# kit4b/kit4b

Measured on AMD Instinct MI355X. Metric: Mreads/sec aligned (100 bp SE vs 3 Gbp .sfx), higher is better.
Workload: dtype u64

## Files before the change

kit4b_amd/csrc/k4_align.hip:

```cpp
#include <stdlib.h>
#include <type_traits>
#include "k4_align_common.h"

#define K4_BS(nch) ((nch) >= 16 ? 128 : 256)
template <int NCH>
struct K4Lane {
  const uint64_t* rd;
  uint32_t* ded;
  const uint32_t* sup;
  const uint64_t* ent;
  uint64_t* memo;
  static constexpr int NW = NCH + 1;
  K4_DEV uint64_t word(int s, int c) const { return rd[(s * NW + c) * K4_BS(NCH)]; }
  K4_DEV uint64_t chunk_at(int s, int o) const {
    int w = o >> 5, sh = 2 * (o & 31);
    uint64_t hi = word(s, w);
    if (!sh) return hi;
    return (hi << sh) | (word(s, w + 1) >> (64 - sh));
  }
};

struct K4Probe {
  int cmp;
  int mm;
  int fm;
  bool exc;
};

#define K4_MEMO_NONE 0ull
K4_DEV uint64_t k4d_memo_pack(int kind, uint64_t pos, int mm, int fm) {
  return ((uint64_t)kind << 62) | ((uint64_t)(fm & 0x3FFF) << 48) | ((uint64_t)(mm & 0xFF) << 40) | (pos & 0xFFFFFFFFFFull);
}

template <int NCH>
K4_DEV K4Probe k4d_probe(const K4DevIndex& ix, const K4Lane<NCH>& ln, int s, int o, int cl, int len, uint64_t p) {
  K4Probe r;
  int64_t left = (int64_t)p - o;
  {
    const int64_t st = left < 0 ? 0 : left;
    const uint64_t b0 = (uint64_t)st >> ix.sup_shift, b1 = (uint64_t)(left + len - 1) >> ix.sup_shift;
    const uint64_t v = (((uint64_t)ln.sup[(b0 >> 5) + 1] << 32) | ln.sup[b0 >> 5]) >> (b0 & 31);
    r.exc = (v & ((2ull << (b1 - b0)) - 1ull)) != 0;
    if (r.exc && ix.sup_shift != K4_EXC_SHIFT) r.exc = k4d_any_exc(ix, left, left + len);
  }
  r.cmp = 0;
  r.mm = 0;
  r.fm = len;
  const uint32_t* wp = ix.ref2 + (left >> 4);
  uint32_t sh = (uint32_t)(left & 15) * 2;
  uint32_t wv[2 * NCH + 1];
  if (NCH <= 5 && len + 15 <= 32 * NCH) {
    uint32_t even[2 * NCH];
    k4d_load_words<2 * NCH>(wp, even);
#pragma unroll
    for (int j = 0; j < 2 * NCH + 1; j++) wv[j] = j < 2 * NCH ? even[j] : 0u;
  } else if (NCH <= 5 || len > 32 * (NCH / 2))
    k4d_load_words<2 * NCH + 1>(wp, wv);
  else {
    uint32_t half[NCH + 1];
    k4d_load_words<NCH + 1>(wp, half);
#pragma unroll
    for (int j = 0; j < 2 * NCH + 1; j++) wv[j] = j < NCH + 1 ? half[j] : 0u;
  }
  bool decided = false;
#pragma unroll
  for (int c = 0; c < NCH; c++) {
    if (32 * c < len) {
      uint64_t hi = ((uint64_t)wv[2 * c] << 32) | wv[2 * c + 1];
      uint64_t refc = sh ? (hi << sh) | (wv[2 * c + 2] >> (32 - sh)) : hi;
      uint64_t rdc = ln.word(s, c);
      uint64_t x = rdc ^ refc;
      const uint64_t xr = x & k4d_range_mask(0, len - 32 * c);
      r.mm += (int)k4d_mm_count(xr);
      if (xr && r.fm == len) r.fm = 32 * c + (__clzll(xr) >> 1);
      uint64_t cm = k4d_range_mask(o - 32 * c, o + cl - 32 * c);
      if (!decided && (x & cm)) {
        r.cmp = (rdc & cm) < (refc & cm) ? -1 : 1;
        decided = true;
      }
    }
  }
  return r;
}

template <int EL, int NCH, typename KT, bool CAPTURE>
K4_DEV int k4d_lcm_fast(const K4AlignArgs& a, const K4Lane<NCH>& ln, int len, int allow_mm, int cl, int core_delta,
                        const K4ReadParams& rp, int* p_inst, int* p_low, int* p_nxt, k4_hit* hits,
                        uint32_t& n_lookup, uint32_t& n_probe, uint32_t& n_cand, bool defer_deep = false) {
  const K4DevIndex& ix = a.ix;
  if (*p_inst > rp.max_hits && *p_low == 0) return K4_HR_HITINSTS;
  if (*p_inst >= 1 && *p_low == 0 && (*p_nxt - *p_low) < rp.mm_delta) return K4_HR_MMDELTA;
  K4State st;
  if (*p_inst <= 0 || *p_low < 0 || *p_nxt < 0) {
    st.inst = *p_inst = 0;
    st.low = *p_low = allow_mm + rp.mm_delta + 1;
    st.nxt = *p_nxt = st.low;
  } else {
    st.inst = *p_inst; st.low = *p_low; st.nxt = *p_nxt;
  }
  st.cur_hit = st.inst < rp.max_hits ? st.inst : -1;
  const int max_iter = ix.max_iter;
  const int64_t n = (int64_t)ix.n;
  const int kk = min((int)ix.k, cl);
  const int tshift = 2 * ((int)ix.k - kk);
  typedef typename std::conditional<EL == 4, uint32_t, KT>::type RT;
  constexpr uint64_t NOPOS = sizeof(RT) == 4 ? 0xFFFFFFFFull : K4_KTAB64_MASK;
  int s = rp.strand == K4_STRAND_CRICK ? 1 : 0;
  const int s_end = rp.strand == K4_STRAND_WATSON ? 0 : 1;
  bool stop = false;
  for (; s <= s_end && !stop; s++) {
    const char strand_c = s ? '-' : '+';
    int n_ded = 0;
    int cur_delta = core_delta;
    int slides = 0;
    int o_next = 0;
    bool more = true;
    bool first_group = true;
    while (more && !stop) {
      constexpr int PFN = NCH == 5 ? K4_PF5 : K4_PF;
      int oo[PFN];
      RT lb0[PFN], ps0[PFN], lb1[PFN];
      uint32_t sig[PFN];
      int cnt = 0;
#pragma unroll
      for (int j = 0; j < PFN; j++) {
        oo[j] = 0; lb0[j] = 0; ps0[j] = 0; lb1[j] = 0; sig[j] = 0;
        if (cnt == j && slides < rp.max_slides && o_next <= len - cl && cur_delta > cl / 3) {
          if (o_next + cl + cur_delta > len) cur_delta = len - (o_next + cl);
          oo[j] = o_next;
          cnt++;
          slides++;
          o_next += cur_delta;
        }
      }
      more = cnt == PFN;
      bool memo_hit = false, memo_pending = false;
      int memo_mm = 0;
#pragma unroll
      for (int j = 0; j < PFN; j++) {
        if (j < cnt) {
          if (!CAPTURE && j == 0 && first_group && tshift == 0 && (sizeof(KT) == 4 || cl >= kk + 2)) {
            const uint64_t mv = ln.memo[s * K4_BS(NCH)];
            const int kind = (int)(mv >> 62), fm = (int)((mv >> 48) & 0x3FFF), mmv = (int)((mv >> 40) & 0xFF);
            if (kind == 1 || (kind == 2 && fm < cl)) continue;
            if (kind == 2 && mmv != 0xFF) {
              lb0[0] = 0; lb1[0] = 1; ps0[0] = (RT)(mv & 0xFFFFFFFFFFull);
              memo_hit = true; memo_mm = mmv;
              continue;
            }
          }
          const uint64_t code = ln.chunk_at(s, oo[j]) >> (64 - 2 * kk);
          uint64_t sub;
          {
            KT e_lb0, e_ps0, e_lb1;
            k4d_ktab_fetch<KT>(ix, code << tshift, (code + 1) << tshift, e_lb0, e_ps0, sig[j], e_lb1, sub,
                               sizeof(KT) == 8 && tshift == 0 && cl >= kk + 2);
            lb0[j] = (RT)e_lb0; ps0[j] = (RT)e_ps0; lb1[j] = (RT)e_lb1;
          }
          if (CAPTURE && defer_deep && tshift == 0 && (uint64_t)(lb1[j] - lb0[j]) > K4_DEFER_BUCKET) return K4_DEFER;
          if (a.deep_general && (!CAPTURE || a.deep_general == 1) && tshift == 0 && (uint64_t)(lb1[j] - lb0[j]) > K4_DEFER_BUCKET) return K4_NEED_SLOW;
          if (sizeof(KT) == 8 && tshift == 0 && cl >= kk + 2 && sub != K4_KTAB64_IRREGULAR) {
            uint32_t before, count;
            k4d_ktab_sub(sub, (uint32_t)(ln.chunk_at(s, oo[j] + kk) >> 60), before, count);
            if (before) ps0[j] = (RT)NOPOS;
            lb0[j] += (RT)before;
            lb1[j] = lb0[j] + (RT)count;
          }
          if (CAPTURE && j == 0 && first_group && tshift == 0) {
            if (lb1[0] == lb0[0]) ln.memo[s * K4_BS(NCH)] = k4d_memo_pack(1, 0, 0, 0);
            else memo_pending = lb1[0] == lb0[0] + 1;
          }
          if (sizeof(KT) == 4 && tshift == 0 && lb1[j] == lb0[j] + 1 && cl > kk) {
            const int nb = min(K4_SIG_BASES32, cl - kk);
            const uint32_t cb = (uint32_t)(ln.chunk_at(s, oo[j] + kk) >> 32);
            const uint32_t df = (cb ^ sig[j]) & (0xFFFFFFFFu << (32 - 2 * nb));
            if (df) {
              lb1[j] = lb0[j];
              if (CAPTURE && j == 0 && first_group) {
                ln.memo[s * K4_BS(NCH)] = k4d_memo_pack(2, (uint64_t)ps0[0], 0xFF, kk + (__clz(df) >> 1));
                memo_pending = false;
              }
            }
          }
        }
      }
      uint32_t touch = 0;
#pragma unroll
      for (int j = 0; j < PFN; j++)
        if (j < cnt && tshift == 0 && lb1[j] > lb0[j] && !(j == 0 && memo_hit) && (sizeof(KT) == 4 || (uint64_t)ps0[j] != NOPOS))
          touch |= ix.ref2[((int64_t)ps0[j] - oo[j]) >> 4];

#pragma unroll
      for (int j = 0; j < PFN; j++) {
        if (j >= cnt || stop) continue;
        const int o = oo[j];
        n_lookup++;
        int64_t lo = (int64_t)lb0[j];
        int64_t hi = (int64_t)lb1[j] - 1;
        const int64_t bucket_hi = hi;
        int64_t found = -1;
        uint64_t fpos = 0;
        int fmm = 0;
        while (lo <= hi) {
          const int64_t mid = (lo + hi) >> 1;
          const uint64_t p = (tshift == 0 && mid == (int64_t)lb0[j] && (sizeof(KT) == 4 || (uint64_t)ps0[j] != NOPOS))
                                 ? (uint64_t)ps0[j] : k4d_sa_at<EL>(ix, (uint64_t)mid);
          K4Probe pr;
          if (!CAPTURE && j == 0 && memo_hit) { pr.cmp = 0; pr.mm = memo_mm; pr.fm = len; pr.exc = false; }
          else {
            pr = k4d_probe<NCH>(ix, ln, s, o, cl, len, p);
            n_probe++;
            if (CAPTURE && j == 0 && memo_pending) ln.memo[s * K4_BS(NCH)] = k4d_memo_pack(2, p, pr.mm > 254 ? 254 : pr.mm, pr.fm);
          }
          if (pr.exc) return K4_NEED_SLOW;
          if (pr.cmp > 0) lo = mid + 1;
          else {
            if (pr.cmp == 0) { found = mid; fpos = p; fmm = pr.mm; }
            hi = mid - 1;
          }
        }
        if (found != lo) continue;
        int64_t idx = found;
        uint64_t p = fpos;
        int mm = fmm;
        int iter = 0;
        bool first = true;
        while (!max_iter || iter < max_iter) {
          if (!first) {
            if (idx >= bucket_hi || idx + 1 >= n) break;
            const uint64_t p2 = k4d_sa_at<EL>(ix, (uint64_t)idx + 1);
            if ((int64_t)p2 + cl > n) break;
            const K4Probe pr = k4d_probe<NCH>(ix, ln, s, o, cl, len, p2);
            n_probe++;
            if (pr.exc) return K4_NEED_SLOW;
            if (pr.cmp != 0) break;
            idx += 1; p = p2; mm = pr.mm;
          }
          first = false;
          if (p < (uint64_t)o) continue;
          const uint64_t left = p - (uint64_t)o;
          int e;
          uint64_t e_start, e_end;
          if (ix.n_entries <= K4_LDS_ENTRIES) {
            int lo_e = 0, hi_e = (int)ix.n_entries - 1;
            e = -1; e_start = 0; e_end = 0;
            while (hi_e >= lo_e) {
              const int mid_e = (hi_e + lo_e) >> 1;
              const uint64_t sv = ln.ent[mid_e];
              if (sv > left) { hi_e = mid_e - 1; continue; }
              const uint64_t ev = ln.ent[K4_LDS_ENTRIES + mid_e];
              if (ev >= left) { e = mid_e; e_start = sv; e_end = ev; break; }
              lo_e = mid_e + 1;
            }
          } else {
            e = k4d_map_entry(ix, left);
            e_start = e >= 0 ? ix.ent_start[e] : 0;
            e_end = e >= 0 ? ix.ent_end[e] : 0;
          }
          if (e < 0 || left + (uint64_t)len - 1 > e_end) continue;
          const uint32_t targ_id = (uint32_t)(1 + p - (uint32_t)o);
          bool dup = false;
          for (int q = 0; q < n_ded; q++) dup |= (ln.ded[q * K4_BS(NCH)] == targ_id);
          if (dup) continue;
          if (n_ded >= K4_DEDUP_CAP) return K4_NEED_SLOW;
          ln.ded[n_ded * K4_BS(NCH)] = targ_id;
          n_ded++;
          iter++;
          n_cand++;
          if (mm > allow_mm || mm >= st.nxt) continue;
          k4d_fold(st, mm, hits, rp.max_hits, ix.ent_id[e], (uint32_t)(left - e_start), len, strand_c);
          if (st.inst > rp.max_hits && st.low == 0) break;
        }
        if (st.inst > rp.max_hits && st.low == 0) stop = true;
      }
      if (touch == 0x5A5A5A5Au && len < 0) n_probe++;
      first_group = false;
    }
  }
  return k4d_lcm_result(*p_inst, *p_low, p_nxt, st, rp.mm_delta, rp.max_hits, p_inst, p_low);
}

K4_DEV uint64_t k4d_rev2(uint64_t x) {
  uint64_t y = __brevll(x);
  return ((y & 0x5555555555555555ull) << 1) | ((y >> 1) & 0x5555555555555555ull);
}

template <int NCH>
K4_DEV uint32_t k4d_pack_read(const uint8_t* __restrict__ src, int len, uint64_t* col, uint32_t& n_ns) {
  constexpr int NW = NCH + 1;
  uint32_t fl = 0;
  n_ns = 0;
  const uint32_t sh = (uint32_t)(reinterpret_cast<uintptr_t>(src) & 3);
  const uint32_t* __restrict__ src32 = reinterpret_cast<const uint32_t*>(src - sh);
  const int span = len + (int)sh;
#pragma unroll
  for (int c = 0; c < NCH; c++) {
    uint64_t acc = 0;
    if (32 * c < len) {
      uint32_t dq[9] = {0, 0, 0, 0, 0, 0, 0, 0, 0};
      if (c * 32 + 32 <= span) {
        uint32_t d8[8];
        k4d_load_words<8>(src32 + c * 8, d8);
#pragma unroll
        for (int q = 0; q < 8; q++) dq[q] = d8[q];
      } else {
#pragma unroll
        for (int q = 0; q < 8; q++)
          if (c * 32 + q * 4 < span) dq[q] = src32[c * 8 + q];
      }
      if (c * 32 + 32 < span) dq[8] = src32[c * 8 + 8];
#pragma unroll
      for (int q = 0; q < 8; q++) {
        const int base = c * 32 + q * 4;
        uint32_t d = __builtin_amdgcn_alignbyte(dq[q + 1], dq[q], sh);
        d &= 0x07070707u;
        if (base + 4 > len) d &= len > base ? (0xFFFFFFFFu >> (8 * (4 - (len - base)))) : 0u;
        const uint32_t hi4 = d & 0x04040404u;
        if (hi4) {
          const uint32_t inval = hi4 & ((d << 1) | (d << 2)) & 0x04040404u;
          if (inval) fl |= K4_RF_INVALID;
          n_ns += __popc(hi4 & ~inval);
          d &= ~(hi4 | (hi4 >> 1) | (hi4 >> 2));
        }
        acc = (acc << 8) | ((d & 3) << 6) | (((d >> 8) & 3) << 4) | (((d >> 16) & 3) << 2) | ((d >> 24) & 3);
      }
    }
    col[c * K4_BS(NCH)] = acc;
  }
  col[NCH * K4_BS(NCH)] = 0;
  if (n_ns) fl |= K4_RF_HAS_N;
#pragma unroll
  for (int c = 0; c < NCH; c++) {
    uint64_t r = 0;
    if (32 * c < len) {
      const int o = len - 32 * (c + 1);
      uint64_t f;
      if (o >= 0) {
        const int w = o >> 5, sh = 2 * (o & 31);
        const uint64_t hi = col[w * K4_BS(NCH)];
        f = sh ? (hi << sh) | (col[(w + 1) * K4_BS(NCH)] >> (64 - sh)) : hi;
      } else
        f = col[0] >> (2 * (-o));
      r = k4d_rev2(~f) & k4d_range_mask(0, len - 32 * c);
    }
    col[(NW + c) * K4_BS(NCH)] = r;
  }
  col[(NW + NCH) * K4_BS(NCH)] = 0;
  return fl;
}

template <int EL, int NCH, bool FIRST, typename KT, bool DEFER = false>
__global__ void __launch_bounds__(K4_BS(NCH), (NCH >= 16 ? K4_STEP_WAVES_LONG : NCH >= 8 ? K4_STEP_WAVES_MID : NCH == 5 ? K4_STEP_WAVES_5 : K4_STEP_WAVES)) k4k_align_step(K4AlignArgs a, int step, const uint32_t* __restrict__ in_ids,
                                                      const uint64_t* __restrict__ in_rows,
                                                      const uint32_t* __restrict__ in_count, uint32_t* __restrict__ out_ids,
                                                      uint64_t* __restrict__ out_rows, uint32_t* __restrict__ out_count) {
  extern __shared__ uint64_t lds[];
  constexpr int NW = NCH + 1;
  const int tid = threadIdx.x;
  const int lane = tid & 63;
  K4Lane<NCH> ln;
  ln.rd = lds + tid;
  ln.ded = reinterpret_cast<uint32_t*>(lds + 2 * NW * K4_BS(NCH)) + tid;
  ln.memo = lds + 2 * NW * K4_BS(NCH) + (K4_DEDUP_CAP * K4_BS(NCH)) / 2 + tid;
  uint64_t* ent_l = lds + 2 * NW * K4_BS(NCH) + (K4_DEDUP_CAP * K4_BS(NCH)) / 2 + 2 * K4_BS(NCH);
  uint32_t* sup_l = reinterpret_cast<uint32_t*>(ent_l + 2 * K4_LDS_ENTRIES);
  ln.ent = ent_l;
  ln.sup = sup_l;
  for (int q = tid; q < K4_SUP_WORDS; q += K4_BS(NCH)) sup_l[q] = a.ix.excsup[q];
  if (a.ix.n_entries <= K4_LDS_ENTRIES)
    for (int q = tid; q < (int)a.ix.n_entries; q += K4_BS(NCH)) {
      ent_l[q] = a.ix.ent_start[q];
      ent_l[K4_LDS_ENTRIES + q] = a.ix.ent_end[q];
    }
  __syncthreads();
  uint64_t* col = lds + tid;
  uint32_t n_lookup = 0, n_probe = 0, n_cand = 0, n_slow = 0, n_bases = 0, n_done = 0;
  const int64_t count = (FIRST && !(DEFER && in_ids != nullptr)) ? a.n_reads : (int64_t)*in_count;
  const int64_t stride = (int64_t)gridDim.x * K4_BS(NCH);
  uint32_t ch_cur = 0, ch_left = 0;
  const bool from_list = !FIRST || (DEFER && in_ids != nullptr);
  const bool may_defer = DEFER && FIRST && in_ids == nullptr && a.defer_ids != nullptr;
  uint32_t dch_cur = 0, dch_left = 0;
  for (int64_t jb = (int64_t)blockIdx.x * K4_BS(NCH) + (tid & ~63); jb < count; jb += stride) {
    const int64_t j = jb + lane;
    bool active = j < count;
    int64_t i = 0;
    if (active) {
      i = from_list ? (int64_t)in_ids[j] : j;
      if (from_list && (uint32_t)i == K4_NO_READ) active = false;
    }
    bool slow = false, survive = false, deferred = false;
    int ext_from = -1;
    if (active) {
      const int len = (int)a.lens[i];
      const K4ReadParams rp = k4d_read_params(a, len);
      bool skip = false;
      if (FIRST) {
        if (!from_list) {
          n_done++;
          n_bases += (uint32_t)len;
        }
        uint32_t fl = 0, n_ns = 0;
        if (len < 1 || len > 32 * NCH || len > K4_MAX_FAST_READ_LEN) {
          fl = K4_RF_TOOLONG;
          if (a.mode == 1) {
            const uint8_t* src = a.reads + a.offs[i];
            for (int q = 0; q < len; q++) {
              uint32_t b = src[q] & 7;
              if (b == 4) n_ns++; else if (b > 4) fl |= K4_RF_INVALID;
            }
          }
        } else
          fl = k4d_pack_read<NCH>(a.reads + a.offs[i], len, col, n_ns);
        if (a.mode == 1) {
          int max_ns = 0;
          if (a.kp.max_ns) max_ns = max((len * a.kp.max_ns) / 100, a.kp.max_ns);
          if ((fl & K4_RF_INVALID) || (int)n_ns > max_ns) {
            k4_read_result r = {K4_HR_SEQERRS, 0, 0, 0, K4_NAR_NS, 0};
            a.rr[i] = r;
            if (!a.sparse_hits)
              for (int q = 0; q < a.max_hits; q++) *reinterpret_cast<uint4*>(&a.hits[i * a.max_hits + q]) = make_uint4(0, 0, 0, 0);
            skip = true;
          }
        }
        slow = fl != 0 && !skip;
        if (((a.mode == 1 && a.kp.pe_mode == 4) || a.best) && !skip) slow = true;
      } else {
        const uint64_t* row = in_rows + (int64_t)j * K4_ROW_WORDS(NCH);
        {
          const k4_u64x2_a8 mv = *reinterpret_cast<const k4_u64x2_a8*>(row + 2 * NCH);
          ln.memo[0] = mv.x; ln.memo[K4_BS(NCH)] = mv.y;
        }
        uint64_t rw[2 * NCH];
#pragma unroll
        for (int c = 0; c < NCH; c++) {
          const k4_u64x2_a8 v = *reinterpret_cast<const k4_u64x2_a8*>(row + 2 * c);
          rw[2 * c] = v.x; rw[2 * c + 1] = v.y;
        }
#pragma unroll
        for (int c = 0; c < NCH; c++) {
          col[c * K4_BS(NCH)] = rw[c];
          col[(NW + c) * K4_BS(NCH)] = rw[NCH + c];
        }
        col[NCH * K4_BS(NCH)] = 0;
        col[(NW + NCH) * K4_BS(NCH)] = 0;
      }
      if (!skip && (rp.core_len < 1 || rp.max_hits < 1 || rp.max_hits > a.max_hits)) slow = true;
      if (!skip && !slow) {
        int n_esc = 0;
        if (rp.tot_mm > 0)
          for (; n_esc <= rp.tot_mm; n_esc++)
            if (len / (n_esc + rp.mm_delta) <= rp.core_len) break;
        const bool has_final = rp.tot_mm > 0 ? n_esc <= rp.tot_mm : true;
        const int n_phases = n_esc + (has_final ? 1 : 0);
        int allow, cl, delta;
        if (step < n_esc) { allow = step; cl = len / (step + rp.mm_delta); delta = cl; }
        else { allow = rp.tot_mm; cl = rp.core_len; delta = rp.core_delta; }
        k4_hit* hits = a.hits + i * a.max_hits;
        int inst = 0, low = 0, nxt = 0;
        const uint32_t c0 = n_lookup, c1 = n_probe, c2 = n_cand;
        if (FIRST) { ln.memo[0] = K4_MEMO_NONE; ln.memo[K4_BS(NCH)] = K4_MEMO_NONE; }
        int rslt = k4d_lcm_fast<EL, NCH, KT, FIRST>(a, ln, len, allow, cl, delta, rp, &inst, &low, &nxt, hits, n_lookup, n_probe, n_cand, DEFER && may_defer);
        if (rslt == K4_NEED_SLOW) {
          slow = true;
          n_lookup = c0; n_probe = c1; n_cand = c2;
        }
        else if (DEFER && rslt == K4_DEFER) {
          deferred = true;
          n_lookup = c0; n_probe = c1; n_cand = c2;
        }
        else if (rslt == 0 && step + 1 >= n_phases && a.ext_on) { slow = true; ext_from = n_phases; }
        else if (rslt != 0 || step + 1 >= n_phases) k4d_finalize(a, i, len, rp, rslt, inst, low, nxt);
        else survive = true;
      }
      if (slow) {
        k4d_push_slow(a, i, ext_from >= 0 ? ext_from : step);
        n_slow++;
      }
    }
    if (FIRST && DEFER) {
      const unsigned long long dm = __ballot(deferred);
      const uint32_t dcnt = (uint32_t)__popcll(dm);
      if (dcnt) {
        if (dcnt > dch_left) {
          for (uint32_t q = lane; q < dch_left; q += 64) a.defer_ids[dch_cur + q] = K4_NO_READ;
          uint32_t base = 0;
          if (lane == 0) base = atomicAdd(&a.ctl[K4_CTL_DEFER], (uint32_t)K4_CHUNK);
          dch_cur = __shfl(base, 0, 64);
          dch_left = K4_CHUNK;
        }
        if (deferred) a.defer_ids[dch_cur + (uint32_t)__popcll(dm & ((1ull << lane) - 1ull))] = (uint32_t)i;
        dch_cur += dcnt;
        dch_left -= dcnt;
      }
    }
    const unsigned long long m = __ballot(survive);
    const uint32_t cnt = (uint32_t)__popcll(m);
    if (cnt) {
      if (cnt > ch_left) {
        for (uint32_t q = lane; q < ch_left; q += 64) out_ids[ch_cur + q] = K4_NO_READ;
        uint32_t base = 0;
        if (lane == 0) base = atomicAdd(out_count, (uint32_t)K4_CHUNK);
        ch_cur = __shfl(base, 0, 64);
        ch_left = K4_CHUNK;
      }
      if (survive) {
        const uint32_t slot = ch_cur + (uint32_t)__popcll(m & ((1ull << lane) - 1ull));
        out_ids[slot] = (uint32_t)i;
        uint64_t* row = out_rows + (int64_t)slot * K4_ROW_WORDS(NCH);
#pragma unroll
        for (int c = 0; c < NCH; c++) {
          k4_u64x2_a8 v;
          const int w0 = 2 * c, w1 = 2 * c + 1;
          v.x = w0 < NCH ? col[w0 * K4_BS(NCH)] : col[(NW + w0 - NCH) * K4_BS(NCH)];
          v.y = w1 < NCH ? col[w1 * K4_BS(NCH)] : col[(NW + w1 - NCH) * K4_BS(NCH)];
          *reinterpret_cast<k4_u64x2_a8*>(row + 2 * c) = v;
        }
        {
          k4_u64x2_a8 mv;
          mv.x = ln.memo[0]; mv.y = ln.memo[K4_BS(NCH)];
          *reinterpret_cast<k4_u64x2_a8*>(row + 2 * NCH) = mv;
        }
      }
      ch_cur += cnt;
      ch_left -= cnt;
    }
  }
  for (uint32_t q = lane; q < ch_left; q += 64) out_ids[ch_cur + q] = K4_NO_READ;
  if (FIRST && DEFER)
    for (uint32_t q = lane; q < dch_left; q += 64) a.defer_ids[dch_cur + q] = K4_NO_READ;
  {
    unsigned long long v[6] = {n_done, n_lookup, n_probe, n_cand, n_slow, n_bases};
#pragma unroll
    for (int q = 0; q < 6; q++) {
      unsigned long long x = v[q];
      for (int d = 32; d > 0; d >>= 1) x += __shfl_down(x, d, 64);
      if (lane == 0 && x) atomicAdd(&a.counters[q], x);
    }
  }
}

static uint32_t next_pow2(uint64_t v) {
  uint32_t p = 1;
  while (p < v) p <<= 1;
  return p;
}

static size_t k4_survivor_slots(size_t cap) {
  static_assert(K4_CHUNK * 7 >= 8 * 63, "cap / 7 must cover the abandoned chunk tails");
  return cap + cap / 7 + (size_t)2048 * 4 * K4_CHUNK + K4_CHUNK;
}

static int nch_for(int max_len) {
  if (max_len <= 128) return 4;
  if (max_len <= 160) return 5;
  if (max_len <= 256) return 8;
  return 16;
}

extern "C" int k4_reserve(k4_index* ix, int64_t max_reads, int32_t max_read_len, int32_t max_hits) {
  if (!ix || max_reads < 0 || max_read_len < 1 || max_hits < 1) return K4_ERR_PARAMS;
  if (max_read_len > K4_MAX_READ_LEN) return k4_fail(ix, K4_ERR_PARAMS, "read length %d exceeds %d", max_read_len, K4_MAX_READ_LEN);
  if (max_reads >= 0xFFFFFFF0ll) return k4_fail(ix, K4_ERR_PARAMS, "at most 2^32-16 reads per batch");
  K4_HIP(ix, hipSetDevice(ix->device));
  K4Workspace& w = ix->ws;
  bool touched = false;
  int fast_len = std::min<int>(max_read_len, K4_MAX_FAST_READ_LEN);
  if (max_reads > w.cap_reads || fast_len > w.cap_len) {
    int64_t cap = std::max<int64_t>(max_reads, w.cap_reads);
    cap = (cap + 255) / 256 * 256;
    int len = std::max(fast_len, w.cap_len);
    int nch = nch_for(len);
    touched = true;
    w.cap_reads = 0;
    w.cap_len = 0;
    const size_t slots = k4_survivor_slots((size_t)cap);
    for (int b = 0; b < 2; b++) {
      K4_HIP(ix, w.ids[b].reserve(slots * 4));
      K4_HIP(ix, w.rows[b].reserve(slots * K4_ROW_WORDS(nch) * 8));
    }
    K4_HIP(ix, w.slow_list.reserve((size_t)cap * 4));
    K4_HIP(ix, w.slow_step.reserve((size_t)cap));
    K4_HIP(ix, w.huge_list.reserve((size_t)cap * 4));
    K4_HIP(ix, w.huge_step.reserve((size_t)cap));
    w.cap_reads = cap;
    w.cap_len = len;
  }
  if (!w.ctl.p) {
    touched = true;
    K4_HIP(ix, w.ctl.reserve(K4_CTL_WORDS * 4));
    K4_HIP(ix, hipMemset(w.ctl.p, 0, K4_CTL_WORDS * 4));
  }
  uint64_t nodes = ix->d.max_iter ? std::min<uint64_t>((uint64_t)ix->d.max_iter * 48, K4_MAX_IDENT_NODES) : K4_MAX_IDENT_NODES;
  uint32_t hcap = next_pow2(std::max<uint64_t>(2 * nodes + 2, 1024));
  if (!w.slow_hash.p || hcap > w.slow_hash_cap) {
    touched = true;
    const size_t words = (size_t)K4_SLOW_WAVES * K4_SMALL_HASH + (size_t)K4_HUGE_WAVES * hcap;
    const size_t bytes = words * 8 + (size_t)(K4_SLOW_WAVES + K4_HUGE_WAVES) * 4;
    K4_HIP(ix, w.slow_hash.reserve(bytes));
    K4_HIP(ix, hipMemset(w.slow_hash.p, 0, bytes));
    w.slow_hash_cap = hcap;
  }
  w.cap_hits = std::max(w.cap_hits, max_hits);
  if (touched) K4_HIP(ix, hipDeviceSynchronize());
  return K4_OK;
}

template <int EL, int NCH, typename KT>
static int launch_steps(k4_index* ix, K4AlignArgs& a, int n_steps, hipStream_t st) {
  K4Workspace& w = ix->ws;
  uint32_t* const ids[2] = {w.ids[0].as<uint32_t>(), w.ids[1].as<uint32_t>()};
  uint64_t* const rows[2] = {w.rows[0].as<uint64_t>(), w.rows[1].as<uint64_t>()};
  uint32_t* const ctl = w.ctl.as<uint32_t>();
  const size_t lds = (size_t)2 * (NCH + 1) * K4_BS(NCH) * 8 + (size_t)K4_DEDUP_CAP * K4_BS(NCH) * 4 + (size_t)2 * K4_BS(NCH) * 8 + (size_t)2 * K4_LDS_ENTRIES * 8 +
                     (size_t)K4_SUP_WORDS * 4 + 16;
  if (lds > 48 * 1024) {
    K4_HIP(ix, hipFuncSetAttribute((const void*)k4k_align_step<EL, NCH, true, KT, false>, hipFuncAttributeMaxDynamicSharedMemorySize, (int)lds));
    K4_HIP(ix, hipFuncSetAttribute((const void*)k4k_align_step<EL, NCH, true, KT, true>, hipFuncAttributeMaxDynamicSharedMemorySize, (int)lds));
    K4_HIP(ix, hipFuncSetAttribute((const void*)k4k_align_step<EL, NCH, false, KT>, hipFuncAttributeMaxDynamicSharedMemorySize, (int)lds));
  }
  const unsigned full = 256 * 8 * (256 / K4_BS(NCH));
  const bool timed = ix->timing && ix->ev_used < 4096;
  if (timed) {
    if (ix->ev_used == ix->ev0.size()) {
      hipEvent_t e0, e1, e2;
      K4_HIP(ix, hipEventCreate(&e0));
      K4_HIP(ix, hipEventCreate(&e1));
      K4_HIP(ix, hipEventCreate(&e2));
      ix->ev0.push_back(e0);
      ix->ev1.push_back(e1);
      ix->ev2.push_back(e2);
    }
    K4_HIP(ix, hipEventRecord(ix->ev0[ix->ev_used], st));
  }
  unsigned grid0 = (unsigned)std::min<int64_t>((a.n_reads + K4_BS(NCH) - 1) / K4_BS(NCH), full);
  static const int deep_mode = getenv("K4_DEEP_TO_GENERAL") ? atoi(getenv("K4_DEEP_TO_GENERAL")) : 0;
  a.deep_general = (deep_mode && ix->deep_bucket_frac >= K4_DEFER_MIN_FRAC) ? deep_mode : 0;
  if (ix->deep_bucket_frac >= K4_DEFER_MIN_FRAC && a.deep_general != 1) {
    a.defer_ids = ids[1];
    hipLaunchKernelGGL((k4k_align_step<EL, NCH, true, KT, true>), dim3(grid0), dim3(K4_BS(NCH)), lds, st, a, 0, (const uint32_t*)nullptr,
                       (const uint64_t*)nullptr, (const uint32_t*)nullptr, ids[0], rows[0], ctl + 2);
    hipLaunchKernelGGL((k4k_align_step<EL, NCH, true, KT, true>), dim3(grid0), dim3(K4_BS(NCH)), lds, st, a, 0, (const uint32_t*)ids[1],
                       (const uint64_t*)nullptr, (const uint32_t*)(ctl + K4_CTL_DEFER), ids[0], rows[0], ctl + 2);
  } else {
    a.defer_ids = nullptr;
    hipLaunchKernelGGL((k4k_align_step<EL, NCH, true, KT, false>), dim3(grid0), dim3(K4_BS(NCH)), lds, st, a, 0, (const uint32_t*)nullptr,
                       (const uint64_t*)nullptr, (const uint32_t*)nullptr, ids[0], rows[0], ctl + 2);
  }
  for (int t = 1; t < n_steps; t++) {
    const int in = (t - 1) & 1, out = t & 1;
    hipLaunchKernelGGL((k4k_align_step<EL, NCH, false, KT>), dim3(grid0), dim3(K4_BS(NCH)), lds, st, a, t, ids[in], rows[in],
                       ctl + 2 + (t - 1), ids[out], rows[out], ctl + 2 + t);
  }
  if (timed) K4_HIP(ix, hipEventRecord(ix->ev1[ix->ev_used], st));
  return K4_OK;
}

template <int EL, typename KT>
static int launch_all(k4_index* ix, K4AlignArgs& a, int max_len, int n_steps, hipStream_t st) {
  K4Workspace& w = ix->ws;
  const int nch = nch_for(std::min(max_len, K4_MAX_FAST_READ_LEN));
  if (nch > nch_for(w.cap_len)) return k4_fail(ix, K4_ERR_INTERNAL, "workspace not reserved for read length %d", max_len);
  if (n_steps < 1 || n_steps > K4_CTL_WORDS - 4) return k4_fail(ix, K4_ERR_INTERNAL, "bad phase count %d", n_steps);
  a.slow_list = w.slow_list.as<uint32_t>();
  a.slow_step = w.slow_step.as<uint8_t>();
  a.ctl = w.ctl.as<uint32_t>();
  a.counters = ix->counters.as<unsigned long long>();
  a.huge_list = w.huge_list.as<uint32_t>();
  a.huge_step = w.huge_step.as<uint8_t>();
  a.slow_hash = w.slow_hash.as<uint64_t>();
  a.slow_hash_cap = w.slow_hash_cap;
  a.slow_gen = reinterpret_cast<uint32_t*>(a.slow_hash + (size_t)K4_SLOW_WAVES * K4_SMALL_HASH + (size_t)K4_HUGE_WAVES * w.slow_hash_cap);
  a.nw = nch + 1;
  if (a.n_reads == 0) return K4_OK;
  K4_HIP(ix, hipMemsetAsync(w.ctl.p, 0, K4_CTL_WORDS * 4, st));
  int rc;
  switch (nch) {
    case 4: rc = launch_steps<EL, 4, KT>(ix, a, n_steps, st); break;
    case 5: rc = launch_steps<EL, 5, KT>(ix, a, n_steps, st); break;
    case 8: rc = launch_steps<EL, 8, KT>(ix, a, n_steps, st); break;
    default: rc = launch_steps<EL, 16, KT>(ix, a, n_steps, st); break;
  }
  if (rc != K4_OK) return rc;
  rc = k4i_launch_general(ix, a, max_len, st);
  if (rc != K4_OK) return rc;
  if (ix->timing && ix->ev_used < ix->ev0.size() && ix->ev_used < 4096) {
    K4_HIP(ix, hipEventRecord(ix->ev2[ix->ev_used], st));
    ix->ev_used++;
  }
  K4_HIP(ix, hipGetLastError());
  return K4_OK;
}

static int run_dev(k4_index* ix, K4AlignArgs& a, int max_len, void* stream) {
  K4Workspace& w = ix->ws;
  if (a.n_reads > w.cap_reads || std::min(max_len, K4_MAX_FAST_READ_LEN) > w.cap_len || a.max_hits > w.cap_hits ||
      !w.slow_hash.p || !w.ids[0].p || !w.ids[1].p || !w.rows[0].p || !w.rows[1].p || !w.slow_list.p || !w.huge_list.p || !w.ctl.p)
    return k4_fail(ix, K4_ERR_PARAMS, "k4_reserve(%lld, %d, %d) must precede the *_dev call", (long long)a.n_reads,
                   max_len, a.max_hits);
  a.ix = ix->d;
  hipStream_t st = (hipStream_t)stream;
  {
    const int mc = a.mode == 0 ? a.ap.min_chimeric_len : a.kp.min_chimeric_len;
    const int mi = a.mode == 0 ? a.ap.micro_indel_len : a.kp.micro_indel_len;
    const int ms = a.mode == 0 ? a.ap.max_splice_junct_len : a.kp.max_splice_junct_len;
    if (mc < 0 || mi < 0 || mi > 20 || ms < 0 || (ms != 0 && (ms < 25 || ms > 100000)))
      return k4_fail(ix, K4_ERR_PARAMS, "MinChimericLen / microInDelLen (0..20) / MaxSpliceJunctLen (0, 25..100000) out of range");
    a.ext_on = (mc > 0 || mi > 0 || ms > 0) ? 1 : 0;
    if ((mi > 0 || ms > 0) && !a.seg2)
      return k4_fail(ix, K4_ERR_PARAMS, "microInDel / splice phases report two segments: use the *_ext entry points (k4_seg2 output)");
    if (a.ext_on && (a.best || (a.mode == 1 && a.kp.pe_mode == 4)))
      return k4_fail(ix, K4_ERR_PARAMS, "the optional AlignReads phases cannot be combined with LocateBestMatches (-N)");
    if (a.seg2 && a.n_reads > 0) K4_HIP(ix, hipMemsetAsync(a.seg2, 0, (size_t)a.n_reads * sizeof(k4_seg2), st));
  }
  int tot_mm = a.ap.tot_mm;
  if (a.mode == 1) {
    tot_mm = a.kp.max_subs == 0 ? 0 : std::max(1, (int)(0.5 + (max_len * a.kp.max_subs) / 100.0));
    tot_mm = std::min(tot_mm, 63);
  }
  const int n_steps = tot_mm + 1;
  if (ix->d.el == 4) return ix->d.ktab64 ? launch_all<4, uint64_t>(ix, a, max_len, n_steps, st) : launch_all<4, uint32_t>(ix, a, max_len, n_steps, st);
  return ix->d.ktab64 ? launch_all<5, uint64_t>(ix, a, max_len, n_steps, st) : launch_all<5, uint32_t>(ix, a, max_len, n_steps, st);
}

static int check_align_params(k4_index* ix, const k4_align_params* p) {
  if (!p) return K4_ERR_PARAMS;
  if (p->tot_mm < 0 || p->tot_mm > 63 || p->core_len < 1 || p->core_delta < 0 || p->max_core_slides < 1 ||
      p->mm_delta < 1 || p->strand < 0 || p->strand > 2 || p->max_hits < 1 || p->max_hits > 4096)
    return k4_fail(ix, K4_ERR_PARAMS, "AlignReads parameters out of range");
  return K4_OK;
}

extern "C" int k4_align_reads_batch_dev(k4_index* ix, const k4_align_params* p, int64_t n, int32_t max_len,
                                        const void* d_reads, const void* d_offs, const void* d_lens, void* d_rslt,
                                        void* d_inst, void* d_low, void* d_nxt, void* d_hits, void* stream) {
  return k4_align_reads_ext_batch_dev(ix, p, n, max_len, d_reads, d_offs, d_lens, d_rslt, d_inst, d_low, d_nxt, d_hits, nullptr, stream);
}
extern "C" int k4_align_reads_ext_batch_dev(k4_index* ix, const k4_align_params* p, int64_t n, int32_t max_len,
                                            const void* d_reads, const void* d_offs, const void* d_lens, void* d_rslt,
                                            void* d_inst, void* d_low, void* d_nxt, void* d_hits, void* d_seg2, void* stream) {
  if (!ix) return K4_ERR_PARAMS;
  int rc = check_align_params(ix, p);
  if (rc != K4_OK) return rc;
  if (n < 0 || (n > 0 && (!d_reads || !d_offs || !d_lens || !d_rslt || !d_inst || !d_low || !d_nxt || !d_hits)))
    return k4_fail(ix, K4_ERR_PARAMS, "null buffer");
  K4AlignArgs a;
  memset(&a, 0, sizeof(a));
  a.reads = (const uint8_t*)d_reads; a.offs = (const uint64_t*)d_offs; a.lens = (const uint32_t*)d_lens;
  a.n_reads = n; a.mode = 0; a.ap = *p;
  a.rslt = (int32_t*)d_rslt; a.inst = (int32_t*)d_inst; a.low = (int32_t*)d_low; a.nxt = (int32_t*)d_nxt;
  a.hits = (k4_hit*)d_hits; a.max_hits = p->max_hits;
  a.seg2 = (k4_seg2*)d_seg2;
  return run_dev(ix, a, max_len, stream);
}

extern "C" int k4_best_matches_batch_dev(k4_index* ix, const k4_align_params* p, int64_t n, int32_t max_len, const void* d_reads,
                                         const void* d_offs, const void* d_lens, void* d_rslt, void* d_inst, void* d_hits,
                                         void* stream) {
  if (!ix) return K4_ERR_PARAMS;
  int rc = check_align_params(ix, p);
  if (rc != K4_OK) return rc;
  if (n < 0 || (n > 0 && (!d_reads || !d_offs || !d_lens || !d_rslt || !d_inst || !d_hits))) return k4_fail(ix, K4_ERR_PARAMS, "null buffer");
  K4AlignArgs a;
  memset(&a, 0, sizeof(a));
  a.reads = (const uint8_t*)d_reads; a.offs = (const uint64_t*)d_offs; a.lens = (const uint32_t*)d_lens;
  a.n_reads = n; a.mode = 0; a.best = 1; a.ap = *p;
  a.rslt = (int32_t*)d_rslt; a.inst = (int32_t*)d_inst;
  a.hits = (k4_hit*)d_hits; a.max_hits = p->max_hits;
  return run_dev(ix, a, max_len, stream);
}

static int resolve_kalign(k4_index* ix, const k4_kalign_params* p, k4_kalign_params* out) {
  if (!p) return K4_ERR_PARAMS;
  *out = *p;
  if (p->max_subs < 0 || p->max_subs > 15 || (p->min_edit_dist != 1 && p->min_edit_dist != 2) || p->max_ns < 0 ||
      p->strand < 0 || p->strand > 2 || p->max_ml < 1 || p->max_ml > 4096 || p->pe_mode < 0 || p->pe_mode > 4)
// ... 249 lines not shown
```

Measured before the change: 3191.

## Extend per-read memo with first two mismatch positions to skip reference probes

Widens the per-strand memo word so it stores the first and second mismatch positions of the first-phase seed alignment. In later phases, probes at the same reference window are settled from the memo: a known mismatch inside the core means no match, and an overlap free of mismatches means a match. This removes reference fetches and compare work in the binary search and in the bucket walk. The cost is an extra second-mismatch scan for surviving reads and a mismatch count now capped at 13, plus a sign-less compare result that is used only when lo == hi.

Measured after the change: 3029. 5.1% lower.

```diff
diff --git a/kit4b_amd/csrc/k4_align.hip b/kit4b_amd/csrc/k4_align.hip
--- a/kit4b_amd/csrc/k4_align.hip
+++ b/kit4b_amd/csrc/k4_align.hip
@@ -1,6 +1,7 @@
 #include <stdlib.h>
 #include <type_traits>
 #include "k4_align_common.h"
+#include "k4_window_memo.h"
 
 #define K4_BS(nch) ((nch) >= 16 ? 128 : 256)
 template <int NCH>
@@ -27,10 +28,6 @@
   bool exc;
 };
 
-#define K4_MEMO_NONE 0ull
-K4_DEV uint64_t k4d_memo_pack(int kind, uint64_t pos, int mm, int fm) {
-  return ((uint64_t)kind << 62) | ((uint64_t)(fm & 0x3FFF) << 48) | ((uint64_t)(mm & 0xFF) << 40) | (pos & 0xFFFFFFFFFFull);
-}
 
 template <int NCH>
 K4_DEV K4Probe k4d_probe(const K4DevIndex& ix, const K4Lane<NCH>& ln, int s, int o, int cl, int len, uint64_t p) {
@@ -81,6 +78,30 @@
     }
   }
   return r;
+}
+
+template <int NCH>
+K4_DEV int k4d_second_mismatch(const K4DevIndex& ix, const K4Lane<NCH>& ln, int s, int len, uint64_t left, int fm) {
+  const uint32_t* wp = ix.ref2 + (left >> 4);
+  const uint32_t sh = (uint32_t)(left & 15) * 2;
+#pragma nounroll
+  for (int c = fm >> 5; 32 * c < len; c++) {
+    const uint64_t hi = ((uint64_t)wp[2 * c] << 32) | wp[2 * c + 1];
+    const uint64_t refc = sh ? (hi << sh) | (wp[2 * c + 2] >> (32 - sh)) : hi;
+    const uint64_t x = (ln.word(s, c) ^ refc) & k4d_range_mask(fm + 1 - 32 * c, len - 32 * c);
+    if (x) return 32 * c + (__clzll(x) >> 1);
+  }
+  return len;
+}
+
+template <int NCH>
+K4_DEV void k4d_memo_complete(const K4DevIndex& ix, const K4Lane<NCH>& ln, int len) {
+#pragma nounroll
+  for (int s = 0; s < 2; s++) {
+    const uint64_t mv = ln.memo[s * K4_BS(NCH)];
+    if (k4wm_has_window(mv) && k4wm_mm(mv) >= 2)
+      ln.memo[s * K4_BS(NCH)] = k4wm_with_p2(mv, k4d_second_mismatch<NCH>(ix, ln, s, len, k4wm_pos(mv), k4wm_p1(mv)));
+  }
 }
 
 template <int EL, int NCH, typename KT, bool CAPTURE>
@@ -135,17 +156,16 @@
       }
       more = cnt == PFN;
       bool memo_hit = false, memo_pending = false;
-      int memo_mm = 0;
 #pragma unroll
       for (int j = 0; j < PFN; j++) {
         if (j < cnt) {
           if (!CAPTURE && j == 0 && first_group && tshift == 0 && (sizeof(KT) == 4 || cl >= kk + 2)) {
             const uint64_t mv = ln.memo[s * K4_BS(NCH)];
-            const int kind = (int)(mv >> 62), fm = (int)((mv >> 48) & 0x3FFF), mmv = (int)((mv >> 40) & 0xFF);
-            if (kind == 1 || (kind == 2 && fm < cl)) continue;
-            if (kind == 2 && mmv != 0xFF) {
-              lb0[0] = 0; lb1[0] = 1; ps0[0] = (RT)(mv & 0xFFFFFFFFFFull);
-              memo_hit = true; memo_mm = mmv;
+            const int kind = k4wm_kind(mv), mmv = k4wm_mm(mv);
+            if (kind == 1 || (kind == 2 && mmv != 0 && k4wm_p1(mv) < cl)) continue;
+            if (kind == 2 && mmv <= K4WM_MM_MAX) {
+              lb0[0] = 0; lb1[0] = 1; ps0[0] = (RT)k4wm_pos(mv);
+              memo_hit = true;
               continue;
             }
           }
@@ -167,7 +187,7 @@
             lb1[j] = lb0[j] + (RT)count;
           }
           if (CAPTURE && j == 0 && first_group && tshift == 0) {
-            if (lb1[0] == lb0[0]) ln.memo[s * K4_BS(NCH)] = k4d_memo_pack(1, 0, 0, 0);
+            if (lb1[0] == lb0[0]) ln.memo[s * K4_BS(NCH)] = k4wm_pack(1, 0, 0, 0, 0);
             else memo_pending = lb1[0] == lb0[0] + 1;
           }
           if (sizeof(KT) == 4 && tshift == 0 && lb1[j] == lb0[j] + 1 && cl > kk) {
@@ -177,7 +197,7 @@
             if (df) {
               lb1[j] = lb0[j];
               if (CAPTURE && j == 0 && first_group) {
-                ln.memo[s * K4_BS(NCH)] = k4d_memo_pack(2, (uint64_t)ps0[0], 0xFF, kk + (__clz(df) >> 1));
+                ln.memo[s * K4_BS(NCH)] = k4wm_pack_unfetched((uint64_t)ps0[0], kk + (__clz(df) >> 1));
                 memo_pending = false;
               }
             }
@@ -187,7 +207,8 @@
       uint32_t touch = 0;
 #pragma unroll
       for (int j = 0; j < PFN; j++)
-        if (j < cnt && tshift == 0 && lb1[j] > lb0[j] && !(j == 0 && memo_hit) && (sizeof(KT) == 4 || (uint64_t)ps0[j] != NOPOS))
+        if (j < cnt && tshift == 0 && lb1[j] > lb0[j] && !(j == 0 && memo_hit) && (sizeof(KT) == 4 || (uint64_t)ps0[j] != NOPOS) &&
+            (CAPTURE || k4wm_decide(ln.memo[s * K4_BS(NCH)], (uint64_t)ps0[j], oo[j], cl) == K4WM_UNDECIDED))
           touch |= ix.ref2[((int64_t)ps0[j] - oo[j]) >> 4];
 
 #pragma unroll
@@ -206,13 +227,16 @@
           const uint64_t p = (tshift == 0 && mid == (int64_t)lb0[j] && (sizeof(KT) == 4 || (uint64_t)ps0[j] != NOPOS))
                                  ? (uint64_t)ps0[j] : k4d_sa_at<EL>(ix, (uint64_t)mid);
           K4Probe pr;
-          if (!CAPTURE && j == 0 && memo_hit) { pr.cmp = 0; pr.mm = memo_mm; pr.fm = len; pr.exc = false; }
+          int known = K4WM_UNDECIDED;
+          if (!CAPTURE && tshift == 0) known = (j == 0 && memo_hit) ? K4WM_MATCH : k4wm_decide(ln.memo[s * K4_BS(NCH)], p, o, cl);
+          if (known == K4WM_MATCH) { pr.cmp = 0; pr.mm = k4wm_mm(ln.memo[s * K4_BS(NCH)]); pr.exc = false; }
+          else if (known == K4WM_NOMATCH && lo == hi) { pr.cmp = K4WM_SIGNLESS_CMP; pr.mm = 0; pr.exc = false; }
           else {
             pr = k4d_probe<NCH>(ix, ln, s, o, cl, len, p);
             n_probe++;
-            if (CAPTURE && j == 0 && memo_pending) ln.memo[s * K4_BS(NCH)] = k4d_memo_pack(2, p, pr.mm > 254 ? 254 : pr.mm, pr.fm);
           }
           if (pr.exc) return K4_NEED_SLOW;
+          if (CAPTURE && j == 0 && memo_pending) ln.memo[s * K4_BS(NCH)] = k4wm_pack_probe(p, pr.mm, pr.fm, 0);
           if (pr.cmp > 0) lo = mid + 1;
           else {
             if (pr.cmp == 0) { found = mid; fpos = p; fmm = pr.mm; }
@@ -230,11 +254,18 @@
             if (idx >= bucket_hi || idx + 1 >= n) break;
             const uint64_t p2 = k4d_sa_at<EL>(ix, (uint64_t)idx + 1);
             if ((int64_t)p2 + cl > n) break;
-            const K4Probe pr = k4d_probe<NCH>(ix, ln, s, o, cl, len, p2);
-            n_probe++;
-            if (pr.exc) return K4_NEED_SLOW;
-            if (pr.cmp != 0) break;
-            idx += 1; p = p2; mm = pr.mm;
+            const int known = (!CAPTURE && tshift == 0) ? k4wm_decide(ln.memo[s * K4_BS(NCH)], p2, o, cl) : K4WM_UNDECIDED;
+            if (known == K4WM_NOMATCH) break;
+            int mm2;
+            if (known == K4WM_MATCH) mm2 = k4wm_mm(ln.memo[s * K4_BS(NCH)]);
+            else {
+              const K4Probe pr = k4d_probe<NCH>(ix, ln, s, o, cl, len, p2);
+              n_probe++;
+              if (pr.exc) return K4_NEED_SLOW;
+              if (pr.cmp != 0) break;
+              mm2 = pr.mm;
+            }
+            idx += 1; p = p2; mm = mm2;
           }
           first = false;
           if (p < (uint64_t)o) continue;
@@ -459,7 +490,7 @@
         k4_hit* hits = a.hits + i * a.max_hits;
         int inst = 0, low = 0, nxt = 0;
         const uint32_t c0 = n_lookup, c1 = n_probe, c2 = n_cand;
-        if (FIRST) { ln.memo[0] = K4_MEMO_NONE; ln.memo[K4_BS(NCH)] = K4_MEMO_NONE; }
+        if (FIRST) { ln.memo[0] = K4WM_NONE; ln.memo[K4_BS(NCH)] = K4WM_NONE; }
         int rslt = k4d_lcm_fast<EL, NCH, KT, FIRST>(a, ln, len, allow, cl, delta, rp, &inst, &low, &nxt, hits, n_lookup, n_probe, n_cand, DEFER && may_defer);
         if (rslt == K4_NEED_SLOW) {
           slow = true;
@@ -471,7 +502,10 @@
         }
         else if (rslt == 0 && step + 1 >= n_phases && a.ext_on) { slow = true; ext_from = n_phases; }
         else if (rslt != 0 || step + 1 >= n_phases) k4d_finalize(a, i, len, rp, rslt, inst, low, nxt);
-        else survive = true;
+        else {
+          survive = true;
+          if (FIRST) k4d_memo_complete<NCH>(a.ix, ln, len);
+        }
       }
       if (slow) {
         k4d_push_slow(a, i, ext_from >= 0 ? ext_from : step);
diff --git a/kit4b_amd/csrc/k4_window_memo.h b/kit4b_amd/csrc/k4_window_memo.h
--- /dev/null
+++ b/kit4b_amd/csrc/k4_window_memo.h
@@ -0,0 +1,46 @@
+#pragma once
+#include <stdint.h>
+
+#if defined(__HIPCC__) || defined(__CUDACC__)
+#define K4WM_FN __host__ __device__ __forceinline__
+#else
+#define K4WM_FN static inline
+#endif
+
+#define K4WM_NONE 0ull
+#define K4WM_MM_MAX 13
+#define K4WM_MM_SAT 14
+#define K4WM_MM_NONE 15
+#define K4WM_POS_MASK 0xFFFFFFFFFFull
+
+#define K4WM_UNDECIDED 0
+#define K4WM_MATCH 1
+#define K4WM_NOMATCH 2
+#define K4WM_SIGNLESS_CMP 1
+
+K4WM_FN uint64_t k4wm_pack(int kind, uint64_t pos, int mm, int p1, int p2) {
+  return ((uint64_t)(kind & 3) << 62) | ((uint64_t)(mm & 15) << 58) | ((uint64_t)(p2 & 0x1FF) << 49) |
+         ((uint64_t)(p1 & 0x1FF) << 40) | (pos & K4WM_POS_MASK);
+}
+K4WM_FN int k4wm_kind(uint64_t w) { return (int)(w >> 62); }
+K4WM_FN int k4wm_mm(uint64_t w) { return (int)((w >> 58) & 15); }
+K4WM_FN int k4wm_p2(uint64_t w) { return (int)((w >> 49) & 0x1FF); }
+K4WM_FN int k4wm_p1(uint64_t w) { return (int)((w >> 40) & 0x1FF); }
+K4WM_FN uint64_t k4wm_pos(uint64_t w) { return w & K4WM_POS_MASK; }
+
+K4WM_FN uint64_t k4wm_pack_probe(uint64_t pos, int mm, int fm, int fm2) {
+  return k4wm_pack(2, pos, mm > K4WM_MM_MAX ? K4WM_MM_SAT : mm, mm >= 1 ? fm : 0, mm >= 2 ? fm2 : 0);
+}
+K4WM_FN uint64_t k4wm_with_p2(uint64_t w, int p2) { return w | ((uint64_t)(p2 & 0x1FF) << 49); }
+K4WM_FN uint64_t k4wm_pack_unfetched(uint64_t pos, int fm) { return k4wm_pack(2, pos, K4WM_MM_NONE, fm, 0); }
+
+K4WM_FN bool k4wm_has_window(uint64_t w) { return k4wm_kind(w) == 2 && k4wm_mm(w) <= K4WM_MM_MAX; }
+
+K4WM_FN int k4wm_decide(uint64_t w, uint64_t p, int o, int cl) {
+  if (!k4wm_has_window(w) || p < (uint64_t)o || p - (uint64_t)o != k4wm_pos(w)) return K4WM_UNDECIDED;
+  const int mm = k4wm_mm(w), p1 = k4wm_p1(w), p2 = k4wm_p2(w);
+  if (mm >= 1 && p1 >= o && p1 < o + cl) return K4WM_NOMATCH;
+  if (mm >= 2 && p2 >= o && p2 < o + cl) return K4WM_NOMATCH;
+  if (mm <= 2 || o + cl - 1 <= p2) return K4WM_MATCH;
+  return K4WM_UNDECIDED;
+}
```
